# AE-HYU/monte_carlo_localization

Hardware: AMD Instinct MI355X
Metric: MCL updates/sec (particle*beam/s) (higher is better)
Workload: dtype f64; 1 GPU; 4194304 particles/GPU x 1081 beams, Spielberg_map (2000x2000 @ 0.05796), initial cloud N((0.0, 0.0, 0.0),(0.5 m,0.5 m,0.4 rad)) (tracking regime), action (0.05, 0.0, 0.01), stock sensor/motion params, multinomial resampling, Philox seed 42; the timed updates follow 5 warm-up updates (the particle set has resampled to motion-noise width); particles_total=4194304, beams=1081, parallelism=single GPU

## Files before the change

include/mcl_hip_engine.h:

```cpp
#ifndef MCL_HIP_ENGINE_H
#define MCL_HIP_ENGINE_H

#include <stddef.h>
#include <stdint.h>

#ifdef __cplusplus
extern "C" {
#endif

#define MCL_ABI_VERSION 1

typedef struct mcl_engine mcl_engine_t;

typedef enum {
    MCL_OK = 0,
    MCL_ERR_INVALID_ARG = -1,
    MCL_ERR_NOT_READY = -2,
    MCL_ERR_HIP = -3,
    MCL_ERR_NO_DEVICE = -4,
    MCL_ERR_UNSUPPORTED = -5,
    MCL_ERR_PEER = -6,
    MCL_ERR_TIMEOUT = -7
} mcl_status;

// ... 69 lines not shown

int mcl_expected_pose(mcl_engine_t *h, double out[3]);

int mcl_get_stage_timings(const mcl_engine_t *h, double ms[6]);

int mcl_get_resample_indices(mcl_engine_t *h, int32_t *idx, int64_t n);
int mcl_get_ray_steps(mcl_engine_t *h, uint8_t *steps, size_t n);
int mcl_get_ray_steps16(mcl_engine_t *h, uint16_t *steps, size_t n);
int mcl_get_log_weights(mcl_engine_t *h, double *logw, int64_t n);
int mcl_get_counters(mcl_engine_t *h, uint64_t out[4]);
int mcl_get_compact_list(const mcl_engine_t *h, int64_t *n_entries, int32_t *used_by_last_update);
int mcl_set_debug_count_probes(mcl_engine_t *h, int32_t on);
int mcl_get_ray_kernel_ms(const mcl_engine_t *h, double *ms);
int mcl_get_ray_kernel_id(const mcl_engine_t *h, int32_t *kernel);
int mcl_get_ray_kernel_variant(const mcl_engine_t *h, int32_t out[3]);
int mcl_get_planned_ray_kernel(const mcl_engine_t *h, int64_t n_particles, int32_t *kernel, const char **reason);
int mcl_get_effective_sample_size(const mcl_engine_t *h, double *n_eff, int32_t *resampled_last_update);

typedef struct {
    int64_t min_particles, max_particles;
    double err;
    double z;
    double bin_x_m, bin_y_m;
    int32_t n_theta_bins;
    int32_t round_to;
    int32_t shrink_permille;
    int32_t reserved;
} mcl_kld_config_t;
void mcl_default_kld_config(mcl_kld_config_t *k);
int mcl_set_kld(mcl_engine_t *h, const mcl_kld_config_t *k);
// ... 249 lines not shown
```

monte_carlo_localization_amd/csrc/mcl_engine.hip:

```cpp
#include "../../include/mcl_hip_engine.h"

#include <hip/hip_runtime.h>
#include <hip/hip_ext.h>
#include <rocprim/device/device_radix_sort.hpp>

#include <algorithm>
#include <chrono>
#include <cmath>
#include <cstdio>
#include <cstring>
#include <string>
#include <vector>

#include "mcl_engine_internal.h"
#include "mcl_kernels.h"
#include "mcl_host_math.h"
#include "mcl_lfield.h"

static_assert(MCL_WEDGES == mcl::kWedges || MCL_KWEDGES != 16, "include/mcl_hip_engine.h and csrc/mcl_wedge.h disagree");

using namespace mcl_host;

namespace {

// ... 66 lines not shown

int sweep_play(const mcl_engine *h, bool hybrid)
{
    if (hybrid) return mcl::kSwSide - (mcl::kSwHybReach + 2) - 3;
    if (h->sweep_global) return 1 << 20;
    return mcl::kSwSide - (h->P + 2) - 3;
}

int64_t max_sweep_units(int64_t n) { return (n + mcl::kSwUnit - 1) / mcl::kSwUnit + mcl::kSwMaxCuts + 2; }

int launch_sweep_plan(mcl_engine *h, int64_t n, int nwg, int g, bool hybrid)
{
    const int ngroups = mcl::kWedges / g;
    MCL_TRY(h->d_items.reserve(h, (size_t)max_sweep_units(n) * ngroups));
    MCL_TRY(h->d_centres.reserve(h, (size_t)max_sweep_units(n)));
    MCL_TRY(h->d_nitems.reserve(h, 1));
    const int play = sweep_play(h, hybrid);
    hipExtLaunchKernelGGL(mcl::k_sweep_plan, dim3(1), dim3(1024), mcl::kPlanLds, h->stream, nullptr, h->ev[EV_K0], 0, h->d_unit_sums.p, h->d_nunits.p, ngroups, nwg,
                          (double)(play / 2 - 1), h->env_sw_guide > 0 ? h->env_sw_guide : (h->sweep_global ? 3 : 2), h->d_items.p, h->d_centres.p, h->d_nitems.p);
    HIPCHK(h, hipGetLastError());
    return MCL_OK;
}

int choose_ray_mode(const mcl_engine *h, int64_t n, bool force_skip, const char **why = nullptr)
{
    const char *dummy;
    const char *&w = why ? *why : dummy;
    const int rk = h->cfg.ray_kernel;
    if (rk == MCL_RAYS_MARCH) { w = "configured: MCL_RAYS_MARCH"; return 1; }
    if (rk == MCL_RAYS_SKIP || force_skip) {
        if (!h->skip_layout_ok) { w = "k_rays_skip's LDS layout check failed at mcl_create: literal march"; return 1; }
        w = force_skip ? "fix-up list overflow: the stage is re-run with k_rays_skip" : "configured: MCL_RAYS_SKIP";
        return 2;
    }
// ... 194 lines not shown
            hipLaunchKernelGGL(mcl::k_hist_partials, dim3(nparts), dim3(256), 0, h->stream, h->d_hist, h->d_histpart, h->d_tile_used);
            hipLaunchKernelGGL(mcl::k_hist_final, dim3(nparts), dim3(256), 0, h->stream, h->d_hist, h->d_histpart, h->d_tile_used);
            hipLaunchKernelGGL(mcl::k_sort_scatter, dim3(nb256), dim3(256), 0, h->stream, h->d_pc, th, n, h->d_skey, h->d_srank,
                               h->d_hist, h->d_pcs, h->d_ths, h->d_perm);
            }
            if (sweep) {
                const size_t mu = (size_t)max_sweep_units(n);
                MCL_TRY(h->d_unit_sums.reserve(h, mu * 2));
                MCL_TRY(h->d_unit_begin.reserve(h, mu + 1));
                MCL_TRY(h->d_nunits.reserve(h, 1));
                hipLaunchKernelGGL(mcl::k_unit_table, dim3(1), dim3(1024), 0, h->stream, h->d_bbox, n, h->d_hist, h->d_histpart, h->d_tile_used,
                                   radix ? h->d_cut_start : (uint32_t *)nullptr, h->d_cut_end, h->d_unit_begin, h->d_nunits, (int)mu);
            }
            if (!radix && !sweep) hipLaunchKernelGGL(mcl::k_hist_clear, dim3(nparts), dim3(256), 0, h->stream, h->d_hist, h->d_tile_used);
            if (sweep) {
                hipLaunchKernelGGL(mcl::k_unit_sums, dim3((unsigned)std::min<int64_t>(max_sweep_units(n), (n + mcl::kSwUnit - 1) / mcl::kSwUnit + 256)), dim3(256), 0, h->stream, h->d_pcs, h->d_unit_begin, h->d_nunits,
                                   h->d_unit_sums, radix ? (uint32_t *)nullptr : h->d_hist, h->d_tile_used, nparts);
            } else {
                MCL_TRY(h->d_slice_mean.reserve(h, (size_t)nsl));
                hipLaunchKernelGGL(mcl::k_slice_means, dim3((unsigned)nsl), dim3(256), 0, h->stream, h->d_pcs, n, (n + nsl - 1) / nsl, h->d_slice_mean);
            }
            a.pcs = h->d_pcs; a.ths = h->d_ths; a.perm = h->d_perm; a.slice_mean = h->d_slice_mean;
            a.distw = h->d_distw; a.distw_stride = (size_t)h->Hp * h->Wps;
        }
        if (h->obs_wait_pending) { h->obs_wait_pending = false; HIPCHK(h, hipStreamWaitEvent(h->stream, h->ev_obs, 0)); }
        if (sweep) {
            if (!h->d_Ltd) return fail(h, MCL_ERR_HIP, "k_rays_sweep: table not allocated (internal)");
            if (!h->ltd_ready) build_ltd(h);
            const int rc_plan = launch_sweep_plan(h, n, nseg, sweep_g, sweep_hyb_now);
            if (rc_plan) return rc_plan;
            a.sweep_g = sweep_g; a.Ltd = h->d_Ltd; a.ltd_cols = h->ltd_cols;
            a.split16 = h->env_sw_split16 >= 0 ? h->env_sw_split16 : 0;
// ... 388 lines not shown
    mcl_engine *h = new mcl_engine();
    h->cfg = *cfg;
    if (const char *e = getenv("MCL_CELL_MIN")) h->env_cell_min = atoll(e);
    if (const char *e = getenv("MCL_CELL_SLICE")) h->env_cell_slice = atoll(e);
    if (const char *e = getenv("MCL_QSLICES_PER_CU")) h->env_qslices_per_cu = atoi(e);
    if (const char *e = getenv("MCL_QSIDE")) h->env_qside = atoi(e);
    if (const char *e = getenv("MCL_SWEEP_G")) h->env_sweep_g = atoi(e);
    if (const char *e = getenv("MCL_TINY_POLL")) h->env_tiny_poll = atoi(e);
    if (const char *e = getenv("MCL_NO_COMPACT")) h->env_no_compact = atoi(e);
    if (const char *e = getenv("MCL_SORT")) h->env_sort_radix = std::strcmp(e, "radix") == 0 ? 1 : (std::strcmp(e, "hist") == 0 ? 0 : -1);
    if (const char *e = getenv("MCL_DEBUG_WG")) h->env_debug_wg = e;
    h->env_no_bucket_cuts = getenv("MCL_NO_BUCKET_CUTS") != nullptr;
    if (const char *e = getenv("MCL_SWEEP_GLOBAL")) h->env_sweep_global = atoi(e) != 0;
    if (const char *e = getenv("MCL_SWEEP_HYBRID")) h->env_sweep_hybrid = atoi(e);
    if (const char *e = getenv("MCL_SW_GUIDE")) h->env_sw_guide = atoi(e);
    if (const char *e = getenv("MCL_SW_SPLIT16")) h->env_sw_split16 = atoi(e) != 0;
    if (const char *e = getenv("MCL_SWEEP_PAIRS")) h->env_sweep_pairs = atoi(e) != 0 ? 1 : 0;
    h->env_no_obs_overlap = getenv("MCL_NO_OBS_OVERLAP") != nullptr;
    h->env_no_prep_fold = getenv("MCL_NO_PREP_FOLD") != nullptr;
    h->env_no_stale_layout = getenv("MCL_NO_STALE_LAYOUT") != nullptr;
    h->env_comm_no_pregather = getenv("MCL_COMM_NO_PREGATHER") != nullptr;
    h->env_comm_no_lists = getenv("MCL_COMM_NO_LISTS") != nullptr;
    h->num_cu = prop.multiProcessorCount;
    h->cap = cfg->max_particles;
    auto bail = [&](const char *what) {
        g_create_error = std::string(what) + ": " + h->err;
        mcl_destroy(h);
        return MCL_ERR_HIP;
    };
#define CRT(call)                                                         \
// ... 70 lines not shown
    CRT(hipFuncSetAttribute(reinterpret_cast<const void *>(&mcl::k_rays_skip<1, true>), hipFuncAttributeMaxDynamicSharedMemorySize, 160 * 1024));
    CRT(hipFuncSetAttribute(reinterpret_cast<const void *>(&mcl::k_rays_skip<1, false>), hipFuncAttributeMaxDynamicSharedMemorySize, 160 * 1024));
    CRT(hipFuncSetAttribute(reinterpret_cast<const void *>(&mcl::k_rays_skip<1, true, true>), hipFuncAttributeMaxDynamicSharedMemorySize, 160 * 1024));
    CRT(hipFuncSetAttribute(reinterpret_cast<const void *>(&mcl::k_rays_skip<1, false, true>), hipFuncAttributeMaxDynamicSharedMemorySize, 160 * 1024));
    CRT(hipFuncSetAttribute(reinterpret_cast<const void *>(&mcl::k_rays_skip<2, false>), hipFuncAttributeMaxDynamicSharedMemorySize, 160 * 1024));
    CRT(hipFuncSetAttribute(reinterpret_cast<const void *>(&mcl::k_rays_skip<3, false>), hipFuncAttributeMaxDynamicSharedMemorySize, 160 * 1024));
    CRT(hipFuncSetAttribute(reinterpret_cast<const void *>(&mcl::k_rays_skip<4, false>), hipFuncAttributeMaxDynamicSharedMemorySize, 160 * 1024));
#ifdef MCL_LEGACY_RAY_KERNELS
    CRT(hipFuncSetAttribute(reinterpret_cast<const void *>(&mcl::k_rays_quad<false>), hipFuncAttributeMaxDynamicSharedMemorySize, 80 * 1024));
    CRT(hipFuncSetAttribute(reinterpret_cast<const void *>(&mcl::k_rays_quad<true>), hipFuncAttributeMaxDynamicSharedMemorySize, 80 * 1024));
    CRT(hipFuncSetAttribute(reinterpret_cast<const void *>(&mcl::k_rays_cell<false>), hipFuncAttributeMaxDynamicSharedMemorySize, 80 * 1024));
    CRT(hipFuncSetAttribute(reinterpret_cast<const void *>(&mcl::k_rays_cell<true>), hipFuncAttributeMaxDynamicSharedMemorySize, 80 * 1024));
#endif
    CRT(hipFuncSetAttribute(reinterpret_cast<const void *>(&mcl::k_tiny_tail<false>), hipFuncAttributeMaxDynamicSharedMemorySize, 64 * 1024));
    CRT(hipFuncSetAttribute(reinterpret_cast<const void *>(&mcl::k_tiny_tail<true>), hipFuncAttributeMaxDynamicSharedMemorySize, 64 * 1024));
    CRT(hipFuncSetAttribute(reinterpret_cast<const void *>(&mcl::k_sweep_plan), hipFuncAttributeMaxDynamicSharedMemorySize, 128 * 1024));
    CRT(hipFuncSetAttribute(reinterpret_cast<const void *>(&mcl::k_rays_sweep<false>), hipFuncAttributeMaxDynamicSharedMemorySize, 80 * 1024));
    CRT(hipFuncSetAttribute(reinterpret_cast<const void *>(&mcl::k_rays_sweep<true>), hipFuncAttributeMaxDynamicSharedMemorySize, 80 * 1024));
    CRT(hipFuncSetAttribute(reinterpret_cast<const void *>(&mcl::k_rays_sweep<false, false, true>), hipFuncAttributeMaxDynamicSharedMemorySize, 80 * 1024 - 64));
    CRT(hipFuncSetAttribute(reinterpret_cast<const void *>(&mcl::k_rays_sweep<true, false, true>), hipFuncAttributeMaxDynamicSharedMemorySize, 80 * 1024 - 64));
    CRT(hipFuncSetAttribute(reinterpret_cast<const void *>(&mcl::k_rays_sweep<false, false, true, true>), hipFuncAttributeMaxDynamicSharedMemorySize, 80 * 1024 - 64));
    CRT(hipFuncSetAttribute(reinterpret_cast<const void *>(&mcl::k_rays_sweep<false, false, true, false, true>), hipFuncAttributeMaxDynamicSharedMemorySize, 80 * 1024 - 64));
    CRT(hipFuncSetAttribute(reinterpret_cast<const void *>(&mcl::k_rays_sweep<true, false, true, false, true>), hipFuncAttributeMaxDynamicSharedMemorySize, 80 * 1024 - 64));
    CRT(hipFuncSetAttribute(reinterpret_cast<const void *>(&mcl::k_rays_sweep<true, false, true, true>), hipFuncAttributeMaxDynamicSharedMemorySize, 80 * 1024 - 64));
    {
        auto static_lds_is = [](const void *fn, size_t want) {
            hipFuncAttributes fa{};
            return hipFuncGetAttributes(&fa, fn) == hipSuccess && fa.sharedSizeBytes == want;
        };
        const size_t qb = (size_t)mcl::kQLdsBase;
        h->sweep_layout_ok = static_lds_is(reinterpret_cast<const void *>(&mcl::k_rays_sweep<false>), qb) && static_lds_is(reinterpret_cast<const void *>(&mcl::k_rays_sweep<true>), qb);
// ... 981 lines not shown
int mcl_get_ray_kernel_ms(const mcl_engine_t *h, double *ms)
{
    if (!h || !ms) return MCL_ERR_INVALID_ARG;
    *ms = h->ray_ms;
    return MCL_OK;
}

int mcl_get_ray_kernel_id(const mcl_engine_t *h, int32_t *kernel)
{
    if (!h || !kernel) return MCL_ERR_INVALID_ARG;
    if (const int rc = lf_refuse_rays(h)) return rc;
    *kernel = h->last_mode;
    return MCL_OK;
}

int mcl_get_ray_kernel_variant(const mcl_engine_t *h, int32_t out[3])
{
    if (!h || !out) return MCL_ERR_INVALID_ARG;
    if (const int rc = lf_refuse_rays(h)) return rc;
    out[0] = h->last_sweep_global; out[1] = h->last_sweep_rec; out[2] = h->last_sweep_pairs;
    return MCL_OK;
}

int mcl_get_planned_ray_kernel(const mcl_engine_t *h, int64_t n_particles, int32_t *kernel, const char **reason)
{
    if (!h || !kernel) return MCL_ERR_INVALID_ARG;
    if (!h->have_map || h->B <= 0) return MCL_ERR_NOT_READY;
    const int64_t n = n_particles > 0 ? n_particles : (h->have_particles ? h->N : h->cap);
    const char *why = "";
    *kernel = choose_ray_mode(h, n, false, &why);
// ... 813 lines not shown
```

monte_carlo_localization_amd/csrc/mcl_engine_internal.h:

```cpp
#pragma once
#include "../../include/mcl_hip_engine.h"

#include <hip/hip_runtime.h>
#include <hip/hip_ext.h>

#include <cstdint>
#include <string>
#include <vector>

#include "mcl_types.h"
#include "mcl_host_math.h"
#include "mcl_buffers.h"

enum { EV_START = 0, EV_RESAMPLE, EV_QUERY, EV_RAYS, EV_SENSOR, EV_K0, EV_K1, EV_COUNT };


constexpr unsigned long long kExactCap = 1ull << 16;
constexpr int kResultWords = 18;
constexpr int kResultStage = 40;
constexpr int kResultStamp = 32;
constexpr int kCompactEntryBytes = 44;

struct mcl_comm;
void comm_free(struct mcl_comm *c);
// ... 62 lines not shown
    int distg_pitch = 0;
    size_t distg_stride = 0;
    const char *distg_why_not = nullptr;
    bool sweep_global = false;
    bool env_sweep_global = false;
    int env_sw_split16 = -1;
    bool env_no_obs_overlap = false;
    bool env_no_prep_fold = false;
    mcl::PrepClear prep_cache{};
    bool prep_cache_valid = false, prep_folded = false;
    int64_t prep_cache_n = 0;
    bool max_partials_ready = false;
    DevBuf<int4> d_items;
    DevBuf<int4> d_centres;
    DevBuf<int> d_nitems;
    int64_t plan_n = 0;
    DevBuf<double4> d_unit_sums;
    DevBuf<uint32_t> d_unit_begin;
    DevBuf<int> d_nunits;
    int64_t env_cell_min = 0, env_cell_slice = 0;
    int env_qslices_per_cu = 0, env_qside = 0, env_sweep_g = 0;
    std::string env_debug_wg;

    int64_t cap = 0, N = 0;
    bool have_particles = false;
    DevBuf<double> d_x[2], d_y[2], d_th[2];
    int cur = 0;
    DevBuf<double> d_w, d_logw, d_tmp;
    DevBuf<double> d_carry[2];
    int carry_idx = 0;
// ... 192 lines not shown
```

monte_carlo_localization_amd/csrc/mcl_rays_sweep.h:

```cpp
#pragma once

namespace mcl {

constexpr int kSwUnder = 127;
constexpr int kSwUnit = 1024;
constexpr int kSwFx = 32;
constexpr int kSwSide = 256;
#ifndef MCL_SW_PITCH
#define MCL_SW_PITCH 260
#endif
constexpr int kSwPitch = MCL_SW_PITCH;
static_assert(kSwPitch >= kSwSide && (kSwPitch % 4) == 0, "window rows are written as dwords");
constexpr int kSwWinBytes = kSwSide * kSwPitch;
#ifndef MCL_SW_HYB_PLAY
#define MCL_SW_HYB_PLAY 40
#endif
constexpr int kSwHybPlay = MCL_SW_HYB_PLAY;
constexpr int kSwHybReach = kSwSide - (kSwHybPlay + 3) - 2;
#if MCL_KWEDGES == 8
__device__ constexpr double kSwHybInvDx[2] = {1.0, 1.414213562373095};
__device__ constexpr double kSwHybInvDy[2] = {1.4142135623730951, 1.0};
#elif MCL_KWEDGES == 16
__device__ constexpr double kSwHybInvDx[4] = {1.0, 1.082392200292394, 1.414213562373095, 2.6131259297527527};
__device__ constexpr double kSwHybInvDy[4] = {2.613125929752753, 1.4142135623730951, 1.082392200292394, 1.0};
// ... 110 lines not shown
                if (b.x + j < (uint32_t)max_units) ub[b.x + j] = b.y + j * kSwUnit;
        }
        if (threadIdx.x == 1023) carry_sh = at + nu;
        __syncthreads();
        if (threadIdx.x == 0) nbig_sh = 0u;
        __syncthreads();
    }
    if (threadIdx.x == 0) {
        int M = (int)carry_sh;
        if (M > max_units) M = max_units;
        ub[M] = (uint32_t)n;
        m_out[0] = M;
    }
}

__global__ __launch_bounds__(256) void k_unit_sums(const double4 *__restrict__ pcs, const uint32_t *__restrict__ ub, const int *__restrict__ m_ptr,
                                                  double4 *__restrict__ out, uint32_t *__restrict__ hist, uint32_t *__restrict__ tile_used, int nparts)
{
    __shared__ double sm[4][7];
    if (hist) {
        for (int t = (int)blockIdx.x; t < nparts; t += (int)gridDim.x) {
            if (!tile_used[t]) continue;
            const uint4 z = make_uint4(0u, 0u, 0u, 0u);
            for (int x = 0; x < kSortXcds; ++x) {
                uint4 *p = reinterpret_cast<uint4 *>(hist + (size_t)x * kSortKeySpace + (size_t)t * kHistTile) + threadIdx.x * 4;
#pragma unroll
                for (int k = 0; k < 4; ++k) p[k] = z;
            }
            __syncthreads();
            if (threadIdx.x == 0) tile_used[t] = 0u;
        }
    }
    for (int u = (int)blockIdx.x; u < m_ptr[0]; u += (int)gridDim.x) {
    if (u != (int)blockIdx.x) __syncthreads();
    const int64_t p_begin = (int64_t)ub[u];
    const int64_t p_end = (int64_t)ub[u + 1];
    double sx = 0.0, sy = 0.0, cnt = 0.0, x0 = INFINITY, x1 = -INFINITY, y0 = INFINITY, y1 = -INFINITY;
    for (int64_t s = p_begin + threadIdx.x; s < p_end; s += blockDim.x) {
        const double4 c = pcs[s];
        if (c.z == c.z && c.w == c.w && fabs(c.z) < 1e9 && fabs(c.w) < 1e9) {
            sx += c.z; sy += c.w; cnt += 1.0;
            x0 = fmin(x0, c.z); x1 = fmax(x1, c.z); y0 = fmin(y0, c.w); y1 = fmax(y1, c.w);
        }
    }
    sx = wave_sum(sx); sy = wave_sum(sy); cnt = wave_sum(cnt);
    x0 = -wave_max(-x0); x1 = wave_max(x1); y0 = -wave_max(-y0); y1 = wave_max(y1);
    const int w = threadIdx.x >> 6;
    if ((threadIdx.x & 63) == 0) { sm[w][0] = sx; sm[w][1] = sy; sm[w][2] = cnt; sm[w][3] = x0; sm[w][4] = x1; sm[w][5] = y0; sm[w][6] = y1; }
    __syncthreads();
    if (threadIdx.x == 0) {
        out[2 * (size_t)u] = make_double4(sm[0][0] + sm[1][0] + sm[2][0] + sm[3][0], sm[0][1] + sm[1][1] + sm[2][1] + sm[3][1],
                                                  sm[0][2] + sm[1][2] + sm[2][2] + sm[3][2], 0.0);
        out[2 * (size_t)u + 1] = make_double4(fmin(fmin(sm[0][3], sm[1][3]), fmin(sm[2][3], sm[3][3])), fmax(fmax(sm[0][4], sm[1][4]), fmax(sm[2][4], sm[3][4])),
                                                      fmin(fmin(sm[0][5], sm[1][5]), fmin(sm[2][5], sm[3][5])), fmax(fmax(sm[0][6], sm[1][6]), fmax(sm[2][6], sm[3][6])));
    }
    }
}

#ifndef MCL_SW_GUIDE
#define MCL_SW_GUIDE 2
#endif
#ifndef MCL_SW_RUNMAX
#define MCL_SW_RUNMAX 16
#endif
constexpr int kSwRunMax = MCL_SW_RUNMAX;
static_assert(kSwRunMax == 16, "k_sweep_plan's bounding-box pyramid has four levels above the units");
constexpr int kPlanBlocks = 256;
constexpr int kPlanLds = (kPlanBlocks * kSwRunMax + kPlanBlocks * kSwRunMax * 15 / 16) * (int)sizeof(float4);
__global__ __launch_bounds__(1024) void k_sweep_plan(const double4 *__restrict__ unit_stats, const int *__restrict__ m_ptr, int ngroups, int nwg, double half_play,
                                                    int guide, int4 *__restrict__ items, int4 *runs, int *__restrict__ nitems_out)
{
    extern __shared__ __attribute__((aligned(16))) unsigned char plan_lds[];
    constexpr int U = kPlanBlocks * kSwRunMax;
    float4 *box0 = reinterpret_cast<float4 *>(plan_lds);
    float4 *pyr = box0 + U;
    __shared__ int wave_tot[4];
    __shared__ int carry_sh;
    const int M = m_ptr[0];
    const int lane = threadIdx.x & 63, wv = threadIdx.x >> 6;
    constexpr int off1 = 0, off2 = U / 2, off3 = off2 + U / 4, off4 = off3 + U / 8;
    const float hp = (float)half_play;
    if (threadIdx.x == 0) carry_sh = 0;
    __syncthreads();
    const int nblocks = (M + kSwRunMax - 1) / kSwRunMax;
    auto unit_box = [&](int u) -> float4 {
        if (u >= M) return make_float4(INFINITY, -INFINITY, INFINITY, -INFINITY);
        const double4 bb = unit_stats[2 * (size_t)u + 1];
        return make_float4((float)bb.x, (float)bb.y, (float)bb.z, (float)bb.w);
    };
    auto join = [](float4 p, float4 q) { return make_float4(fminf(p.x, q.x), fmaxf(p.y, q.y), fminf(p.z, q.z), fmaxf(p.w, q.w)); };
    for (int b0 = 0; b0 < nblocks; b0 += kPlanBlocks) {
        const int ubase = b0 * kSwRunMax;
        const int ucnt = min(U, ((M - ubase + kSwRunMax - 1) / kSwRunMax) * kSwRunMax);
        for (int k = threadIdx.x; k < ucnt; k += 1024) box0[k] = unit_box(ubase + k);
        __syncthreads();
        for (int k = threadIdx.x; k < ucnt / 2; k += 1024) pyr[off1 + k] = join(box0[2 * k], box0[2 * k + 1]);
        __syncthreads();
        for (int k = threadIdx.x; k < ucnt / 4; k += 1024) pyr[off2 + k] = join(pyr[off1 + 2 * k], pyr[off1 + 2 * k + 1]);
        __syncthreads();
        for (int k = threadIdx.x; k < ucnt / 8; k += 1024) pyr[off3 + k] = join(pyr[off2 + 2 * k], pyr[off2 + 2 * k + 1]);
        __syncthreads();
        for (int k = threadIdx.x; k < ucnt / 16; k += 1024) pyr[off4 + k] = join(pyr[off3 + 2 * k], pyr[off3 + 2 * k + 1]);
        __syncthreads();
        auto run_box = [&](int r, int cc) -> float4 {
            return cc == 1 ? box0[r] : cc == 2 ? pyr[off1 + (r >> 1)] : cc == 4 ? pyr[off2 + (r >> 2)] : cc == 8 ? pyr[off3 + (r >> 3)] : pyr[off4 + (r >> 4)];
        };
        const int b = b0 + (int)threadIdx.x;
        const int u0 = b * kSwRunMax, r0 = (int)threadIdx.x * kSwRunMax;
        const bool mine = (int)threadIdx.x < kPlanBlocks && b < nblocks;
        unsigned int starts = 0u;
        int nruns = 0;
        if (mine) {
            long long want = ((long long)(M - u0) * ngroups) / ((long long)(guide > 0 ? guide : MCL_SW_GUIDE) * (nwg > 0 ? nwg : 1));
            int c = 1;
            while (c * 2 <= kSwRunMax && c * 2 <= want) c *= 2;
            for (int k0 = 0; k0 < kSwRunMax && u0 + k0 < M; k0 += c) {
                int cc = c;
                int k = k0;
                while (k < k0 + c && u0 + k < M) {
                    bool fits = true;
                    if (cc > 1) {
                        const float4 bb = run_box(r0 + k, cc);
                        if (bb.y >= bb.x) fits = 0.5f * (bb.y - bb.x) < hp && 0.5f * (bb.w - bb.z) < hp;
                    }
                    if (fits || cc == 1) { starts |= 1u << k; ++nruns; k += cc; }
                    else cc >>= 1;
                }
            }
        }
        int inc = nruns;
#pragma unroll
        for (int o = 1; o < 64; o <<= 1) { const int t = __shfl_up(inc, o, 64); if (lane >= o) inc += t; }
        if (lane == 63 && wv < 4) wave_tot[wv] = inc;
        __syncthreads();
        const int at_base = carry_sh;
        int at = at_base + inc - nruns;
        for (int k = 0; k < wv && k < 4; ++k) at += wave_tot[k];
        if (mine) {
            const int uend = (u0 + kSwRunMax < M) ? kSwRunMax : M - u0;
            unsigned int rest = starts;
            while (rest) {
                const int k = __ffs((int)rest) - 1;
                rest &= rest - 1u;
                const int knext = rest ? __ffs((int)rest) - 1 : uend;
                const int len = knext - k;
                int cc = 1;
                while (cc < len) cc <<= 1;
                const float4 bb = run_box(r0 + k, cc);
                const float mx = bb.y >= bb.x ? 0.5f * (bb.x + bb.y) : 0.0f, my = bb.y >= bb.x ? 0.5f * (bb.z + bb.w) : 0.0f;
                runs[at++] = make_int4((int)floorf(mx) + 1, (int)floorf(my) + 1, u0 + k, len);
            }
        }
        __syncthreads();
        if ((int)threadIdx.x == kPlanBlocks - 1) carry_sh = at;
        __syncthreads();
        const int nr = carry_sh - at_base;
        for (int idx = threadIdx.x; idx < nr * ngroups; idx += 1024) {
            const int r = at_base + idx / ngroups, g = idx - (idx / ngroups) * ngroups;
            const int4 rn = runs[r];
            items[(size_t)r * ngroups + g] = make_int4(rn.z, rn.w, (g + rn.z) % ngroups, r);
        }
        __syncthreads();
    }
    if (threadIdx.x == 0) nitems_out[0] = carry_sh * ngroups;
}

#define MCL_SW_TRIP(REM, GIN, BYIN, TXIN, TYIN, TX, TY, TXLO, TXHI, TYLO, TYHI, AD, BY, GOUT, REMOUT, XX, XY, LB) \
    "v_mad_u64_u32 " TX ", vcc, " BYIN ", " XX ", " TXIN "\n\t"                                           \
    "v_mad_u64_u32 " TY ", vcc, " BYIN ", " XY ", " TYIN "\n\t"                                           \
    "v_mad_u32_u24 " AD ", " TYHI ", %[wp], " TXHI "\n\t"                                                 \
    "ds_read_i8 " BY ", " AD " offset:" LB "\n\t"                                                         \
    "v_min3_u32 " GOUT ", " GIN ", " TXLO ", " TYLO "\n\t"                                                \
    "s_waitcnt lgkmcnt(0)\n\t"                                                                            \
    "v_sub_co_u32 " REMOUT ", vcc, " REM ", " BY "\n\t"                                                   \
    "s_andn2_b64 exec, exec, vcc\n\t"

#define MCL_SW_DIR_TAB(NEGA, NEGB)                                                                                              \
        "s_waitcnt vmcnt(1)\n\t"                                      \
        "v_fma_f64 v[48:49], -%[bq], v[42:43], %[magic1]\n\t"                                                                  \
// ... 712 lines not shown
```

monte_carlo_localization_amd/engine.py:

```python
from __future__ import annotations

import ctypes as C
import os

import numpy as np

_HERE = os.path.dirname(os.path.abspath(__file__))
LIB_PATH = os.environ.get("MCL_LIB") or os.path.join(_HERE, "libmcl_hip_engine.so")

MCL_OK = 0
MCL_ERR_INVALID_ARG = -1
MCL_ERR_NOT_READY = -2
MCL_ERR_PEER = -6
MCL_ERR_TIMEOUT = -7
RESAMPLE_MULTINOMIAL, RESAMPLE_SYSTEMATIC = 0, 1
WEIGHT_LOG, WEIGHT_PRODUCT = 0, 1
RAYS_AUTO, RAYS_MARCH, RAYS_SKIP, RAYS_QUAD, RAYS_CELL, RAYS_SWEEP = 0, 1, 2, 3, 4, 5
BUF_X, BUF_Y, BUF_THETA, BUF_QWEIGHT, BUF_LOGW, BUF_SCALARS = range(6)

EXPORTS = [
    "mcl_abi_version", "mcl_default_config", "mcl_create", "mcl_destroy", "mcl_last_error", "mcl_set_map",
    "mcl_get_max_range_px", "mcl_get_sensor_table", "mcl_set_beam_angles", "mcl_set_particles",
    "mcl_get_particles", "mcl_get_weights", "mcl_sample_particles", "mcl_particle_mean", "mcl_update",
    "mcl_sensor_update", "mcl_expected_pose", "mcl_get_stage_timings", "mcl_get_resample_indices",
    "mcl_get_ray_steps", "mcl_get_log_weights", "mcl_get_counters", "mcl_get_ray_kernel_ms", "mcl_device_ptr",
    "mcl_stage_propagate", "mcl_stage_weights", "mcl_stage_finish", "mcl_scan_weights", "mcl_export_state",
    "mcl_get_scalars", "mcl_host_sensor_table", "mcl_host_skip_field", "mcl_init_particles_pose", "mcl_init_global",
    "mcl_update_scan", "mcl_get_ray_kernel_id", "mcl_host_skip_field_dir", "mcl_host_skip_field_wedge", "mcl_export_records", "mcl_get_effective_sample_size", "mcl_get_host_scalars", "mcl_stage_resample_records", "mcl_stage_resample", "mcl_stage_rays",
    "mcl_set_reserved_cus", "mcl_stage_resample_indices", "mcl_stage_motion_records", "mcl_stage_distinct_parents", "mcl_export_records_at",
    "mcl_group_create", "mcl_group_destroy", "mcl_group_last_error", "mcl_group_size", "mcl_group_engine", "mcl_group_set_map",
    "mcl_group_set_beam_angles", "mcl_group_set_particles", "mcl_group_init_particles_pose", "mcl_group_init_global",
    "mcl_group_update", "mcl_group_expected_pose", "mcl_group_get_particles", "mcl_group_get_weights",
    "mcl_group_get_resample_indices", "mcl_group_get_stage_timings", "mcl_group_exchange_bytes",
    "mcl_set_debug_count_probes", "mcl_set_particles_shard", "mcl_get_compact_list", "mcl_compact_chunk_bytes", "mcl_export_compact",
    "mcl_stage_resample_compact", "mcl_group_exchanged_lists", "mcl_get_ray_steps16", "mcl_get_planned_ray_kernel",
    "mcl_stream_wait_external", "mcl_external_wait_stream", "mcl_export_compact_async", "mcl_stage_resample_compact_async",
    "mcl_stage_rays_async", "mcl_stage_weights_async", "mcl_stage_complete", "mcl_stage_keep",
    "mcl_comm_available", "mcl_comm_unique_id", "mcl_comm_create", "mcl_comm_destroy", "mcl_comm_update", "mcl_comm_stats", "mcl_comm_set_lists", "mcl_comm_get_vector", "mcl_comm_last_exchange", "mcl_comm_selftest",
    "mcl_host_sweep_global_layout", "mcl_get_ray_kernel_variant",
    "mcl_default_kld_config", "mcl_set_kld", "mcl_get_particle_count", "mcl_get_kld_state", "mcl_host_kld_bins", "mcl_host_kld_target",
    "mcl_default_cluster_config", "mcl_pose_clusters", "mcl_get_cluster_labels",
    "mcl_query_scans", "mcl_score_poses", "mcl_get_query_counters",
    "mcl_default_search_config", "mcl_global_search", "mcl_get_search_scores", "mcl_get_search_bytes", "mcl_host_search_lattice",
    "mcl_host_search_headings", "mcl_init_particles_mixture",
    "mcl_global_search_sequence", "mcl_host_search_sequence_offsets", "mcl_host_relative_poses",
    "mcl_default_search_stream_config", "mcl_global_search_streamed", "mcl_host_search_slabs",
    "mcl_global_search_beam", "mcl_host_search_beam_grid", "mcl_get_search_beam_table",
    "mcl_default_refine_config", "mcl_refine_poses", "mcl_get_refine_scores", "mcl_get_refine_bytes", "mcl_host_refine_window",
    "mcl_host_refine_reduce",
    "mcl_default_recovery_config", "mcl_set_recovery", "mcl_get_recovery_state", "mcl_set_recovery_state", "mcl_host_recovery_step",
    "mcl_default_likelihood_field_config", "mcl_set_likelihood_field", "mcl_get_likelihood_field", "mcl_get_likelihood_table",
    "mcl_host_likelihood_field", "mcl_host_likelihood_table",
    "mcl_default_motion_config", "mcl_set_motion_model", "mcl_get_motion_model", "mcl_host_motion_scalars", "mcl_host_motion_sample",
    "mcl_init_particles_gaussian", "mcl_host_gaussian_factor", "mcl_group_set_motion_model", "mcl_group_init_particles_gaussian",
# ... 988 lines not shown
    def effective_sample_size(self):
        v, r = C.c_double(), C.c_int32()
        self._chk(self.lib.mcl_get_effective_sample_size(self._h, C.byref(v), C.byref(r)), "mcl_get_effective_sample_size")
        return v.value, bool(r.value)

    def ray_kernel_name(self):
        v = C.c_int32()
        self._chk(self.lib.mcl_get_ray_kernel_id(self._h, C.byref(v)), "mcl_get_ray_kernel_id")
        return {1: "k_rays_march", 2: "k_rays_skip", 3: "k_rays_quad", 4: "k_rays_cell", 5: "k_rays_sweep"}.get(v.value, "?")

    def ray_kernel_variant(self):
        v = (C.c_int32 * 3)()
        self._chk(self.lib.mcl_get_ray_kernel_variant(self._h, v), "mcl_get_ray_kernel_variant")
        return dict(global_fields=v[0] == 1, hybrid=v[0] == 2, turned_directions=bool(v[1]), pairs=bool(v[2]))

    RAY_KERNEL_NAMES = {0: None, 1: "k_rays_march", 2: "k_rays_skip", 3: "k_rays_quad", 4: "k_rays_cell", 5: "k_rays_sweep"}

    def planned_ray_kernel(self, n_particles=0):
        v, why = C.c_int32(), C.c_char_p()
        self._chk(self.lib.mcl_get_planned_ray_kernel(self._h, C.c_int64(int(n_particles)), C.byref(v), C.byref(why)), "mcl_get_planned_ray_kernel")
        return self.RAY_KERNEL_NAMES.get(v.value, "?"), (why.value or b"").decode()

    def device_ptr(self, which) -> int:
        p = C.c_void_p()
        self._chk(self.lib.mcl_device_ptr(self._h, C.c_int32(which), C.byref(p)), "mcl_device_ptr")
        return int(p.value or 0)

    def export_state(self, d_x=0, d_y=0, d_th=0, d_q=0):
        self._chk(self.lib.mcl_export_state(self._h, C.c_void_p(d_x or None), C.c_void_p(d_y or None),
                                            C.c_void_p(d_th or None), C.c_void_p(d_q or None)), "mcl_export_state")
# ... 300 lines not shown
```

Baseline: 868.3 billion particle*beam/s.

## Cull sweep work items for wedge groups no particle heading can reach

k_unit_sums now computes, per sweep unit, a bitmask of direction wedges touched by any particle's beam fan, based on its heading and the first and last beam angles. k_sweep_plan propagates these masks through its bounding-box pyramid. It emits work items only for run/group pairs whose wedge group is live, compacting the item list with a 64-bit packed prefix scan. The aim is to skip sweep work for wedge groups that no particle's beams cover, at the cost of extra heading reads, mask reductions and more LDS in the plan kernel (fewer plan blocks when there are more than 32 wedges). Diagnostic getters for the plan counts and unit masks are also added.

Measured after the change: 869.6 billion particle*beam/s (median of 6 runs). About the same (+0.2%).

```diff
diff --git a/include/mcl_hip_engine.h b/include/mcl_hip_engine.h
--- a/include/mcl_hip_engine.h
+++ b/include/mcl_hip_engine.h
@@ -107,6 +107,9 @@
 int mcl_get_ray_kernel_ms(const mcl_engine_t *h, double *ms);
 int mcl_get_ray_kernel_id(const mcl_engine_t *h, int32_t *kernel);
 int mcl_get_ray_kernel_variant(const mcl_engine_t *h, int32_t out[3]);
+int mcl_get_sweep_plan_counts(mcl_engine_t *h, int64_t out[2]);
+int mcl_get_sweep_units(mcl_engine_t *h, int32_t *n_units, uint32_t *unit_begin, uint64_t *wedge_masks, size_t max_units,
+                        double *sorted_theta, int64_t n);
 int mcl_get_planned_ray_kernel(const mcl_engine_t *h, int64_t n_particles, int32_t *kernel, const char **reason);
 int mcl_get_effective_sample_size(const mcl_engine_t *h, double *n_eff, int32_t *resampled_last_update);
 
diff --git a/monte_carlo_localization_amd/csrc/mcl_engine.hip b/monte_carlo_localization_amd/csrc/mcl_engine.hip
--- a/monte_carlo_localization_amd/csrc/mcl_engine.hip
+++ b/monte_carlo_localization_amd/csrc/mcl_engine.hip
@@ -104,10 +104,12 @@
     const int ngroups = mcl::kWedges / g;
     MCL_TRY(h->d_items.reserve(h, (size_t)max_sweep_units(n) * ngroups));
     MCL_TRY(h->d_centres.reserve(h, (size_t)max_sweep_units(n)));
-    MCL_TRY(h->d_nitems.reserve(h, 1));
+    MCL_TRY(h->d_run_live.reserve(h, (size_t)max_sweep_units(n)));
+    MCL_TRY(h->d_nitems.reserve(h, 2));
     const int play = sweep_play(h, hybrid);
     hipExtLaunchKernelGGL(mcl::k_sweep_plan, dim3(1), dim3(1024), mcl::kPlanLds, h->stream, nullptr, h->ev[EV_K0], 0, h->d_unit_sums.p, h->d_nunits.p, ngroups, nwg,
-                          (double)(play / 2 - 1), h->env_sw_guide > 0 ? h->env_sw_guide : (h->sweep_global ? 3 : 2), h->d_items.p, h->d_centres.p, h->d_nitems.p);
+                          (double)(play / 2 - 1), h->env_sw_guide > 0 ? h->env_sw_guide : (h->sweep_global ? 3 : 2), h->env_sweep_no_cull ? 0 : 1, h->d_items.p, h->d_centres.p,
+                          h->d_run_live.p, h->d_nitems.p);
     HIPCHK(h, hipGetLastError());
     return MCL_OK;
 }
@@ -332,8 +334,8 @@
             }
             if (!radix && !sweep) hipLaunchKernelGGL(mcl::k_hist_clear, dim3(nparts), dim3(256), 0, h->stream, h->d_hist, h->d_tile_used);
             if (sweep) {
-                hipLaunchKernelGGL(mcl::k_unit_sums, dim3((unsigned)std::min<int64_t>(max_sweep_units(n), (n + mcl::kSwUnit - 1) / mcl::kSwUnit + 256)), dim3(256), 0, h->stream, h->d_pcs, h->d_unit_begin, h->d_nunits,
-                                   h->d_unit_sums, radix ? (uint32_t *)nullptr : h->d_hist, h->d_tile_used, nparts);
+                hipLaunchKernelGGL(mcl::k_unit_sums, dim3((unsigned)std::min<int64_t>(max_sweep_units(n), (n + mcl::kSwUnit - 1) / mcl::kSwUnit + 256)), dim3(256), 0, h->stream, h->d_pcs, h->d_ths, h->d_unit_begin, h->d_nunits,
+                                   a.beam_a0, a.beam_alast, h->d_unit_sums, radix ? (uint32_t *)nullptr : h->d_hist, h->d_tile_used, nparts);
             } else {
                 MCL_TRY(h->d_slice_mean.reserve(h, (size_t)nsl));
                 hipLaunchKernelGGL(mcl::k_slice_means, dim3((unsigned)nsl), dim3(256), 0, h->stream, h->d_pcs, n, (n + nsl - 1) / nsl, h->d_slice_mean);
@@ -752,6 +754,7 @@
     if (const char *e = getenv("MCL_SWEEP_GLOBAL")) h->env_sweep_global = atoi(e) != 0;
     if (const char *e = getenv("MCL_SWEEP_HYBRID")) h->env_sweep_hybrid = atoi(e);
     if (const char *e = getenv("MCL_SW_GUIDE")) h->env_sw_guide = atoi(e);
+    if (const char *e = getenv("MCL_SWEEP_NO_CULL")) h->env_sweep_no_cull = atoi(e) != 0;
     if (const char *e = getenv("MCL_SW_SPLIT16")) h->env_sw_split16 = atoi(e) != 0;
     if (const char *e = getenv("MCL_SWEEP_PAIRS")) h->env_sweep_pairs = atoi(e) != 0 ? 1 : 0;
     h->env_no_obs_overlap = getenv("MCL_NO_OBS_OVERLAP") != nullptr;
@@ -852,7 +855,7 @@
 #endif
     CRT(hipFuncSetAttribute(reinterpret_cast<const void *>(&mcl::k_tiny_tail<false>), hipFuncAttributeMaxDynamicSharedMemorySize, 64 * 1024));
     CRT(hipFuncSetAttribute(reinterpret_cast<const void *>(&mcl::k_tiny_tail<true>), hipFuncAttributeMaxDynamicSharedMemorySize, 64 * 1024));
-    CRT(hipFuncSetAttribute(reinterpret_cast<const void *>(&mcl::k_sweep_plan), hipFuncAttributeMaxDynamicSharedMemorySize, 128 * 1024));
+    CRT(hipFuncSetAttribute(reinterpret_cast<const void *>(&mcl::k_sweep_plan), hipFuncAttributeMaxDynamicSharedMemorySize, mcl::kPlanLds));
     CRT(hipFuncSetAttribute(reinterpret_cast<const void *>(&mcl::k_rays_sweep<false>), hipFuncAttributeMaxDynamicSharedMemorySize, 80 * 1024));
     CRT(hipFuncSetAttribute(reinterpret_cast<const void *>(&mcl::k_rays_sweep<true>), hipFuncAttributeMaxDynamicSharedMemorySize, 80 * 1024));
     CRT(hipFuncSetAttribute(reinterpret_cast<const void *>(&mcl::k_rays_sweep<false, false, true>), hipFuncAttributeMaxDynamicSharedMemorySize, 80 * 1024 - 64));
@@ -1864,6 +1867,46 @@
     return MCL_OK;
 }
 
+int mcl_get_sweep_plan_counts(mcl_engine_t *h, int64_t out[2])
+{
+    if (!h || !out) return MCL_ERR_INVALID_ARG;
+    if (const int rc = lf_refuse_rays(h)) return rc;
+    if (h->last_mode != 5 || !h->d_nitems) return fail(h, MCL_ERR_NOT_READY, "the last ray stage did not run k_rays_sweep");
+    int v[2] = {0, 0};
+    HIPCHK(h, hipSetDevice(h->cfg.device));
+    HIPCHK(h, hipMemcpyAsync(v, h->d_nitems, sizeof(v), hipMemcpyDeviceToHost, h->stream));
+    HIPCHK(h, hipStreamSynchronize(h->stream));
+    out[0] = v[0]; out[1] = v[1];
+    return MCL_OK;
+}
+
+int mcl_get_sweep_units(mcl_engine_t *h, int32_t *n_units, uint32_t *unit_begin, uint64_t *wedge_masks, size_t max_units, double *sorted_theta,
+                        int64_t n)
+{
+    if (!h || !n_units) return MCL_ERR_INVALID_ARG;
+    if (const int rc = lf_refuse_rays(h)) return rc;
+    if (h->last_mode != 5 || !h->d_nunits || !h->d_unit_begin || !h->d_unit_sums) return fail(h, MCL_ERR_NOT_READY, "the last ray stage did not run k_rays_sweep");
+    HIPCHK(h, hipSetDevice(h->cfg.device));
+    int M = 0;
+    HIPCHK(h, hipMemcpyAsync(&M, h->d_nunits, sizeof(int), hipMemcpyDeviceToHost, h->stream));
+    HIPCHK(h, hipStreamSynchronize(h->stream));
+    *n_units = M;
+    if (unit_begin || wedge_masks) {
+        if (M < 0 || max_units < (size_t)M) return fail(h, MCL_ERR_INVALID_ARG, "room for fewer units than the sorted order has");
+        if (unit_begin) HIPCHK(h, hipMemcpyAsync(unit_begin, h->d_unit_begin, ((size_t)M + 1) * sizeof(uint32_t), hipMemcpyDeviceToHost, h->stream));
+        if (wedge_masks && M > 0) {
+            HIPCHK(h, hipMemcpy2DAsync(wedge_masks, sizeof(uint64_t), reinterpret_cast<const char *>(h->d_unit_sums.p) + 24, 2 * sizeof(double4), sizeof(uint64_t),
+                                       (size_t)M, hipMemcpyDeviceToHost, h->stream));
+        }
+    }
+    if (sorted_theta) {
+        if (n != h->N) return fail(h, MCL_ERR_INVALID_ARG, "n is not the particle count");
+        HIPCHK(h, hipMemcpyAsync(sorted_theta, h->d_ths, (size_t)n * sizeof(double), hipMemcpyDeviceToHost, h->stream));
+    }
+    HIPCHK(h, hipStreamSynchronize(h->stream));
+    return MCL_OK;
+}
+
 int mcl_get_ray_kernel_variant(const mcl_engine_t *h, int32_t out[3])
 {
     if (!h || !out) return MCL_ERR_INVALID_ARG;
diff --git a/monte_carlo_localization_amd/csrc/mcl_engine_internal.h b/monte_carlo_localization_amd/csrc/mcl_engine_internal.h
--- a/monte_carlo_localization_amd/csrc/mcl_engine_internal.h
+++ b/monte_carlo_localization_amd/csrc/mcl_engine_internal.h
@@ -100,6 +100,8 @@
     DevBuf<int4> d_items;
     DevBuf<int4> d_centres;
     DevBuf<int> d_nitems;
+    DevBuf<int4> d_run_live;
+    bool env_sweep_no_cull = false;
     int64_t plan_n = 0;
     DevBuf<double4> d_unit_sums;
     DevBuf<uint32_t> d_unit_begin;
diff --git a/monte_carlo_localization_amd/csrc/mcl_rays_sweep.h b/monte_carlo_localization_amd/csrc/mcl_rays_sweep.h
--- a/monte_carlo_localization_amd/csrc/mcl_rays_sweep.h
+++ b/monte_carlo_localization_amd/csrc/mcl_rays_sweep.h
@@ -148,10 +148,30 @@
     }
 }
 
-__global__ __launch_bounds__(256) void k_unit_sums(const double4 *__restrict__ pcs, const uint32_t *__restrict__ ub, const int *__restrict__ m_ptr,
-                                                  double4 *__restrict__ out, uint32_t *__restrict__ hist, uint32_t *__restrict__ tile_used, int nparts)
+#if MCL_KWEDGES > 32
+typedef unsigned long long SwMask;
+#else
+typedef unsigned int SwMask;
+#endif
+constexpr SwMask kSwMaskAll = (SwMask)~(SwMask)0 >> (sizeof(SwMask) * 8 - kWedges);
+__device__ __forceinline__ SwMask sweep_wedge_mask(double th, double beam_a0, double beam_alast)
+{
+    if (!(th == th && fabs(th) < 1e6)) return (SwMask)1;
+    const int w0 = beam_wedge_d(th, beam_a0), wl = beam_wedge_d(th, beam_alast);
+    const int cnt = wl - w0 + 1;
+    if (cnt <= 0) return (SwMask)0;
+    if (cnt >= kWedges) return kSwMaskAll;
+    const SwMask base = ((SwMask)1 << cnt) - (SwMask)1;
+    const int s = w0 & (kWedges - 1);
+    return ((base << s) | (s ? base >> (kWedges - s) : (SwMask)0)) & kSwMaskAll;
+}
+
+__global__ __launch_bounds__(256) void k_unit_sums(const double4 *__restrict__ pcs, const double *__restrict__ ths, const uint32_t *__restrict__ ub, const int *__restrict__ m_ptr,
+                                                  double beam_a0, double beam_alast, double4 *__restrict__ out, uint32_t *__restrict__ hist,
+                                                  uint32_t *__restrict__ tile_used, int nparts)
 {
     __shared__ double sm[4][7];
+    __shared__ SwMask smm[4];
     if (hist) {
         for (int t = (int)blockIdx.x; t < nparts; t += (int)gridDim.x) {
             if (!tile_used[t]) continue;
@@ -170,8 +190,10 @@
     const int64_t p_begin = (int64_t)ub[u];
     const int64_t p_end = (int64_t)ub[u + 1];
     double sx = 0.0, sy = 0.0, cnt = 0.0, x0 = INFINITY, x1 = -INFINITY, y0 = INFINITY, y1 = -INFINITY;
+    SwMask wm = 0;
     for (int64_t s = p_begin + threadIdx.x; s < p_end; s += blockDim.x) {
         const double4 c = pcs[s];
+        wm |= sweep_wedge_mask(ths[s], beam_a0, beam_alast);
         if (c.z == c.z && c.w == c.w && fabs(c.z) < 1e9 && fabs(c.w) < 1e9) {
             sx += c.z; sy += c.w; cnt += 1.0;
             x0 = fmin(x0, c.z); x1 = fmax(x1, c.z); y0 = fmin(y0, c.w); y1 = fmax(y1, c.w);
@@ -179,12 +201,15 @@
     }
     sx = wave_sum(sx); sy = wave_sum(sy); cnt = wave_sum(cnt);
     x0 = -wave_max(-x0); x1 = wave_max(x1); y0 = -wave_max(-y0); y1 = wave_max(y1);
+#pragma unroll
+    for (int o = 32; o > 0; o >>= 1) wm |= (SwMask)__shfl_xor(wm, o, 64);
     const int w = threadIdx.x >> 6;
-    if ((threadIdx.x & 63) == 0) { sm[w][0] = sx; sm[w][1] = sy; sm[w][2] = cnt; sm[w][3] = x0; sm[w][4] = x1; sm[w][5] = y0; sm[w][6] = y1; }
+    if ((threadIdx.x & 63) == 0) { sm[w][0] = sx; sm[w][1] = sy; sm[w][2] = cnt; sm[w][3] = x0; sm[w][4] = x1; sm[w][5] = y0; sm[w][6] = y1; smm[w] = wm; }
     __syncthreads();
     if (threadIdx.x == 0) {
         out[2 * (size_t)u] = make_double4(sm[0][0] + sm[1][0] + sm[2][0] + sm[3][0], sm[0][1] + sm[1][1] + sm[2][1] + sm[3][1],
-                                                  sm[0][2] + sm[1][2] + sm[2][2] + sm[3][2], 0.0);
+                                                  sm[0][2] + sm[1][2] + sm[2][2] + sm[3][2],
+                                                  __longlong_as_double((long long)(unsigned long long)(smm[0] | smm[1] | smm[2] | smm[3])));
         out[2 * (size_t)u + 1] = make_double4(fmin(fmin(sm[0][3], sm[1][3]), fmin(sm[2][3], sm[3][3])), fmax(fmax(sm[0][4], sm[1][4]), fmax(sm[2][4], sm[3][4])),
                                                       fmin(fmin(sm[0][5], sm[1][5]), fmin(sm[2][5], sm[3][5])), fmax(fmax(sm[0][6], sm[1][6]), fmax(sm[2][6], sm[3][6])));
     }
@@ -199,24 +224,29 @@
 #endif
 constexpr int kSwRunMax = MCL_SW_RUNMAX;
 static_assert(kSwRunMax == 16, "k_sweep_plan's bounding-box pyramid has four levels above the units");
-constexpr int kPlanBlocks = 256;
-constexpr int kPlanLds = (kPlanBlocks * kSwRunMax + kPlanBlocks * kSwRunMax * 15 / 16) * (int)sizeof(float4);
+constexpr int kPlanBlocks = kWedges > 32 ? 128 : 256;
+constexpr int kPlanLds = (kPlanBlocks * kSwRunMax + kPlanBlocks * kSwRunMax * 15 / 16) * (int)(sizeof(float4) + sizeof(SwMask));
+static_assert(kPlanLds + 64 <= 160 * 1024, "k_sweep_plan's pass must fit the LDS of a CU");
 __global__ __launch_bounds__(1024) void k_sweep_plan(const double4 *__restrict__ unit_stats, const int *__restrict__ m_ptr, int ngroups, int nwg, double half_play,
-                                                    int guide, int4 *__restrict__ items, int4 *runs, int *__restrict__ nitems_out)
+                                                    int guide, int cull, int4 *__restrict__ items, int4 *runs, int4 *run_live, int *__restrict__ nitems_out)
 {
     extern __shared__ __attribute__((aligned(16))) unsigned char plan_lds[];
     constexpr int U = kPlanBlocks * kSwRunMax;
     float4 *box0 = reinterpret_cast<float4 *>(plan_lds);
     float4 *pyr = box0 + U;
-    __shared__ int wave_tot[4];
-    __shared__ int carry_sh;
+    SwMask *umask = reinterpret_cast<SwMask *>(pyr + U * 15 / 16);
+    SwMask *mpyr = umask + U;
+    __shared__ long long wave_tot[4];
+    __shared__ int carry_sh, carry_items_sh;
     const int M = m_ptr[0];
     const int lane = threadIdx.x & 63, wv = threadIdx.x >> 6;
     constexpr int off1 = 0, off2 = U / 2, off3 = off2 + U / 4, off4 = off3 + U / 8;
     const float hp = (float)half_play;
-    if (threadIdx.x == 0) carry_sh = 0;
+    if (threadIdx.x == 0) { carry_sh = 0; carry_items_sh = 0; }
     __syncthreads();
     const int nblocks = (M + kSwRunMax - 1) / kSwRunMax;
+    const int G = kWedges / ngroups;
+    const unsigned long long all_groups = ~0ull >> (64 - ngroups);
     auto unit_box = [&](int u) -> float4 {
         if (u >= M) return make_float4(INFINITY, -INFINITY, INFINITY, -INFINITY);
         const double4 bb = unit_stats[2 * (size_t)u + 1];
@@ -226,24 +256,37 @@
     for (int b0 = 0; b0 < nblocks; b0 += kPlanBlocks) {
         const int ubase = b0 * kSwRunMax;
         const int ucnt = min(U, ((M - ubase + kSwRunMax - 1) / kSwRunMax) * kSwRunMax);
-        for (int k = threadIdx.x; k < ucnt; k += 1024) box0[k] = unit_box(ubase + k);
-        __syncthreads();
-        for (int k = threadIdx.x; k < ucnt / 2; k += 1024) pyr[off1 + k] = join(box0[2 * k], box0[2 * k + 1]);
-        __syncthreads();
-        for (int k = threadIdx.x; k < ucnt / 4; k += 1024) pyr[off2 + k] = join(pyr[off1 + 2 * k], pyr[off1 + 2 * k + 1]);
-        __syncthreads();
-        for (int k = threadIdx.x; k < ucnt / 8; k += 1024) pyr[off3 + k] = join(pyr[off2 + 2 * k], pyr[off2 + 2 * k + 1]);
-        __syncthreads();
-        for (int k = threadIdx.x; k < ucnt / 16; k += 1024) pyr[off4 + k] = join(pyr[off3 + 2 * k], pyr[off3 + 2 * k + 1]);
+        for (int k = threadIdx.x; k < ucnt; k += 1024) {
+            box0[k] = unit_box(ubase + k);
+            umask[k] = ubase + k < M ? (SwMask)(unsigned long long)__double_as_longlong(unit_stats[2 * (size_t)(ubase + k)].w) : (SwMask)0;
+        }
+        __syncthreads();
+        for (int k = threadIdx.x; k < ucnt / 2; k += 1024) { pyr[off1 + k] = join(box0[2 * k], box0[2 * k + 1]); mpyr[off1 + k] = umask[2 * k] | umask[2 * k + 1]; }
+        __syncthreads();
+        for (int k = threadIdx.x; k < ucnt / 4; k += 1024) { pyr[off2 + k] = join(pyr[off1 + 2 * k], pyr[off1 + 2 * k + 1]); mpyr[off2 + k] = mpyr[off1 + 2 * k] | mpyr[off1 + 2 * k + 1]; }
+        __syncthreads();
+        for (int k = threadIdx.x; k < ucnt / 8; k += 1024) { pyr[off3 + k] = join(pyr[off2 + 2 * k], pyr[off2 + 2 * k + 1]); mpyr[off3 + k] = mpyr[off2 + 2 * k] | mpyr[off2 + 2 * k + 1]; }
+        __syncthreads();
+        for (int k = threadIdx.x; k < ucnt / 16; k += 1024) { pyr[off4 + k] = join(pyr[off3 + 2 * k], pyr[off3 + 2 * k + 1]); mpyr[off4 + k] = mpyr[off3 + 2 * k] | mpyr[off3 + 2 * k + 1]; }
         __syncthreads();
         auto run_box = [&](int r, int cc) -> float4 {
             return cc == 1 ? box0[r] : cc == 2 ? pyr[off1 + (r >> 1)] : cc == 4 ? pyr[off2 + (r >> 2)] : cc == 8 ? pyr[off3 + (r >> 3)] : pyr[off4 + (r >> 4)];
+        };
+        auto run_groups = [&](int r, int cc) -> unsigned long long {
+            if (!cull) return all_groups;
+            const unsigned long long wm = cc == 1 ? umask[r] : cc == 2 ? mpyr[off1 + (r >> 1)] : cc == 4 ? mpyr[off2 + (r >> 2)] : cc == 8 ? mpyr[off3 + (r >> 3)] : mpyr[off4 + (r >> 4)];
+            if (G == 1) return wm;
+            unsigned long long gm = 0ull;
+            for (int gg = 0; gg < ngroups; ++gg)
+                if ((wm >> (gg * G)) & (G >= 64 ? ~0ull : (1ull << G) - 1ull)) gm |= 1ull << gg;
+            return gm;
         };
         const int b = b0 + (int)threadIdx.x;
         const int u0 = b * kSwRunMax, r0 = (int)threadIdx.x * kSwRunMax;
         const bool mine = (int)threadIdx.x < kPlanBlocks && b < nblocks;
         unsigned int starts = 0u;
         int nruns = 0;
+        int nlive = 0;
         if (mine) {
             long long want = ((long long)(M - u0) * ngroups) / ((long long)(guide > 0 ? guide : MCL_SW_GUIDE) * (nwg > 0 ? nwg : 1));
             int c = 1;
@@ -257,21 +300,24 @@
                         const float4 bb = run_box(r0 + k, cc);
                         if (bb.y >= bb.x) fits = 0.5f * (bb.y - bb.x) < hp && 0.5f * (bb.w - bb.z) < hp;
                     }
-                    if (fits || cc == 1) { starts |= 1u << k; ++nruns; k += cc; }
+                    if (fits || cc == 1) { starts |= 1u << k; ++nruns; nlive += __popcll(run_groups(r0 + k, cc)); k += cc; }
                     else cc >>= 1;
                 }
             }
         }
-        int inc = nruns;
+        const int uend = (u0 + kSwRunMax < M) ? kSwRunMax : M - u0;
+        const long long mine_cnt = ((long long)nruns << 32) | (long long)nlive;
+        long long inc = mine_cnt;
 #pragma unroll
-        for (int o = 1; o < 64; o <<= 1) { const int t = __shfl_up(inc, o, 64); if (lane >= o) inc += t; }
+        for (int o = 1; o < 64; o <<= 1) { const long long t = __shfl_up(inc, o, 64); if (lane >= o) inc += t; }
         if (lane == 63 && wv < 4) wave_tot[wv] = inc;
         __syncthreads();
         const int at_base = carry_sh;
-        int at = at_base + inc - nruns;
-        for (int k = 0; k < wv && k < 4; ++k) at += wave_tot[k];
+        long long before = inc - mine_cnt;
+        for (int k = 0; k < wv && k < 4; ++k) before += wave_tot[k];
+        int at = at_base + (int)(before >> 32);
+        int item_at = carry_items_sh + (int)(before & 0xFFFFFFFFll);
         if (mine) {
-            const int uend = (u0 + kSwRunMax < M) ? kSwRunMax : M - u0;
             unsigned int rest = starts;
             while (rest) {
                 const int k = __ffs((int)rest) - 1;
@@ -282,21 +328,28 @@
                 while (cc < len) cc <<= 1;
                 const float4 bb = run_box(r0 + k, cc);
                 const float mx = bb.y >= bb.x ? 0.5f * (bb.x + bb.y) : 0.0f, my = bb.y >= bb.x ? 0.5f * (bb.z + bb.w) : 0.0f;
+                const unsigned long long live = run_groups(r0 + k, cc);
+                run_live[at] = make_int4(item_at, 0, (int)(unsigned int)live, (int)(unsigned int)(live >> 32));
+                item_at += __popcll(live);
                 runs[at++] = make_int4((int)floorf(mx) + 1, (int)floorf(my) + 1, u0 + k, len);
             }
         }
         __syncthreads();
-        if ((int)threadIdx.x == kPlanBlocks - 1) carry_sh = at;
+        if ((int)threadIdx.x == kPlanBlocks - 1) { carry_sh = at; carry_items_sh = item_at; }
         __syncthreads();
         const int nr = carry_sh - at_base;
         for (int idx = threadIdx.x; idx < nr * ngroups; idx += 1024) {
             const int r = at_base + idx / ngroups, g = idx - (idx / ngroups) * ngroups;
             const int4 rn = runs[r];
-            items[(size_t)r * ngroups + g] = make_int4(rn.z, rn.w, (g + rn.z) % ngroups, r);
-        }
-        __syncthreads();
-    }
-    if (threadIdx.x == 0) nitems_out[0] = carry_sh * ngroups;
+            const int4 lv = run_live[r];
+            const unsigned long long live = ((unsigned long long)(unsigned int)lv.w << 32) | (unsigned long long)(unsigned int)lv.z;
+            const int s = rn.z % ngroups;
+            const unsigned long long rot = ((live >> s) | (s ? live << (ngroups - s) : 0ull)) & all_groups;
+            if ((rot >> g) & 1ull) items[(size_t)lv.x + __popcll(rot & ((1ull << g) - 1ull))] = make_int4(rn.z, rn.w, (g + rn.z) % ngroups, r);
+        }
+        __syncthreads();
+    }
+    if (threadIdx.x == 0) { nitems_out[0] = carry_items_sh; nitems_out[1] = carry_sh * ngroups; }
 }
 
 #define MCL_SW_TRIP(REM, GIN, BYIN, TXIN, TYIN, TX, TY, TXLO, TXHI, TYLO, TYHI, AD, BY, GOUT, REMOUT, XX, XY, LB) \
diff --git a/monte_carlo_localization_amd/engine.py b/monte_carlo_localization_amd/engine.py
--- a/monte_carlo_localization_amd/engine.py
+++ b/monte_carlo_localization_amd/engine.py
@@ -37,7 +37,7 @@
     "mcl_stream_wait_external", "mcl_external_wait_stream", "mcl_export_compact_async", "mcl_stage_resample_compact_async",
     "mcl_stage_rays_async", "mcl_stage_weights_async", "mcl_stage_complete", "mcl_stage_keep",
     "mcl_comm_available", "mcl_comm_unique_id", "mcl_comm_create", "mcl_comm_destroy", "mcl_comm_update", "mcl_comm_stats", "mcl_comm_set_lists", "mcl_comm_get_vector", "mcl_comm_last_exchange", "mcl_comm_selftest",
-    "mcl_host_sweep_global_layout", "mcl_get_ray_kernel_variant",
+    "mcl_host_sweep_global_layout", "mcl_get_ray_kernel_variant", "mcl_get_sweep_plan_counts", "mcl_get_sweep_units",
     "mcl_default_kld_config", "mcl_set_kld", "mcl_get_particle_count", "mcl_get_kld_state", "mcl_host_kld_bins", "mcl_host_kld_target",
     "mcl_default_cluster_config", "mcl_pose_clusters", "mcl_get_cluster_labels",
     "mcl_query_scans", "mcl_score_poses", "mcl_get_query_counters",
@@ -1056,6 +1056,19 @@
         self._chk(self.lib.mcl_get_ray_kernel_variant(self._h, v), "mcl_get_ray_kernel_variant")
         return dict(global_fields=v[0] == 1, hybrid=v[0] == 2, turned_directions=bool(v[1]), pairs=bool(v[2]))
 
+    def sweep_plan_counts(self):
+        v = (C.c_int64 * 2)()
+        self._chk(self.lib.mcl_get_sweep_plan_counts(self._h, v), "mcl_get_sweep_plan_counts")
+        return int(v[0]), int(v[1])
+
+    def sweep_units(self):
+        m = C.c_int32()
+        self._chk(self.lib.mcl_get_sweep_units(self._h, C.byref(m), None, None, C.c_size_t(0), None, C.c_int64(0)), "mcl_get_sweep_units")
+        ub, wm, th = np.empty(m.value + 1, np.uint32), np.empty(m.value, np.uint64), np.empty(self.n, np.float64)
+        self._chk(self.lib.mcl_get_sweep_units(self._h, C.byref(m), _p(ub), _p(wm), C.c_size_t(m.value), _p(th), C.c_int64(self.n)),
+                  "mcl_get_sweep_units")
+        return ub, wm, th
+
     RAY_KERNEL_NAMES = {0: None, 1: "k_rays_march", 2: "k_rays_skip", 3: "k_rays_quad", 4: "k_rays_cell", 5: "k_rays_sweep"}
 
     def planned_ray_kernel(self, n_particles=0):
```
